# sandyresearch/chipmunk

Hardware: AMD Instinct MI355X
Metric: DiT denoise steps/sec at fixed sparsity (higher is better)
Workload: dtype bf16

## Files before the change

chipmunk_amd/csrc/attn96.hip:

```cpp
#include "common.h"
#include "attn64_regs.h"
#include "attn_params.h"
#include "attn64_util.h"
#include "attn96_sched.h"

namespace {

constexpr int KT = 32;
constexpr int TB = KT * 256;
constexpr int NSL = 4;
constexpr int VRING = NSL * TB;
constexpr int QLDS = 2 * NSL * TB;
constexpr int LDS_BYTES = QLDS + 2 * 8192;
constexpr float SCALE_LOG2E = 0.08838834764f * 1.44269504089f;
constexpr float MAX_LAG = 4.0f;
#ifndef A96_ABL
#define A96_ABL 0
#endif

template <int QB, int DB>
__device__ __forceinline__ void mfma_pv(const u32x4 &vf, const u32x4 &pf) {
    constexpr int oa = (QB * 4 + DB) * 16;
    asm volatile("s_nop 4\n\tv_mfma_f32_32x32x16_bf16 a[%c2:%c3], %0, %1, a[%c2:%c3]" ::"v"(vf), "v"(pf), "i"(oa), "i"(oa + 15));
}
template <int KS, int SLOT>
__device__ __forceinline__ void lds_k(uint32_t addr) {
    constexpr int ka = 192 + KS * 4;
    asm volatile("ds_read_b128 a[%c1:%c2], %0 offset:%c3" ::"v"(addr), "i"(ka), "i"(ka + 3), "i"(SLOT * TB) : "memory");
}

#ifdef ATTN96_PROF
__device__ unsigned long long g_a96_prof[2 * 8];
#define P96_DECL unsigned long long pt_ = 0, pacc_[7] = {0, 0, 0, 0, 0, 0, 0}; const bool prof_on_ = blockIdx.x == 700
#define P96_START() do { if (prof_on_) pt_ = __builtin_amdgcn_s_memtime(); } while (0)
#define P96_MARK(i) do { if (prof_on_) { const unsigned long long n_ = __builtin_amdgcn_s_memtime(); pacc_[i] += n_ - pt_; pt_ = n_; } } while (0)
#define P96_END(w, n) do { if (prof_on_ && lane == 0) { for (int i_ = 0; i_ < 7; ++i_) g_a96_prof[(w) * 8 + i_] = pacc_[i_]; g_a96_prof[(w) * 8 + 7] = (n); } } while (0)
#else
#define P96_DECL
#define P96_START()
#define P96_MARK(i)
#define P96_END(w, n)
#endif

template <bool INPLACE>
__global__ __launch_bounds__(128) __attribute__((amdgpu_waves_per_eu(1, 1))) void csp96_kernel(const AttnParams p) {
    extern __shared__ __attribute__((aligned(16))) unsigned char smem[];
    const int tid = threadIdx.x, lane = tid & 63;
    const int w = __builtin_amdgcn_readfirstlane(tid >> 6);
    const int l31 = lane & 31, hf = lane >> 5, l15 = lane & 15, lg = lane >> 4;
#ifdef ATTN96_PROF
    const unsigned long long t_entry_ = __builtin_amdgcn_s_memtime();
#endif
    int wid = blockIdx.x;
    const int wid0 = wid;
    wid = p.plan[2 * wid0];
    if (wid < 0) return;
    const int meta = p.plan[2 * wid0 + 1];
    const int sp = meta & 0xff, nsp = (meta >> 8) & 0xff;
    const int slot0 = meta >> 16, tix = meta >> 16;
    const int bh = wid / p.G, g = wid - bh * p.G;
    const int b = bh / p.H, h = bh - b * p.H;
    const int row0 = g * 192 + w * 96;
    const int count = p.counts[(int64_t)bh * p.G + g];
    const int valid = count < p.Nk ? count : p.Nk;
    const int ntiles_all = (valid + KT - 1) / KT;
    const int tbeg = (int)((int64_t)ntiles_all * sp / nsp), tend = (int)((int64_t)ntiles_all * (sp + 1) / nsp);
    const int ntiles = tend - tbeg;
    const int T4 = (ntiles + 3) & ~3;

    const uint16_t *kbase = p.k + b * p.ks[0] + h * p.ks[1];
    const uint16_t *vbase = p.v + b * p.vs[0] + h * p.vs[1];
    const __amdgpu_buffer_rsrc_t krsrc = make_rsrc(kbase), vrsrc = make_rsrc(vbase);
    const uint32_t kstride_b = (uint32_t)p.ks[2] * 2u, vstride_b = (uint32_t)p.vs[2] * 2u;
    const IndexRow irow = index_row(p, (int64_t)bh * p.G + g);
    const int32_t *idx = irow.ptr;

    const uint32_t lds0 = (uint32_t)(uintptr_t)(__attribute__((address_space(3))) unsigned char *)smem;
    uint32_t kad[8];
#pragma unroll
    for (int ks = 0; ks < 8; ++ks) kad[ks] = lds0 + l31 * 256 + (((2 * ks + hf) ^ l15) << 4);
    const uint32_t qad = lds0 + QLDS + w * 8192 + l31 * 256;
    uint32_t vad[4];
#pragma unroll
    for (int db = 0; db < 4; ++db)
        vad[db] = lds0 + VRING + (4 * hf + (l15 >> 2)) * 256 + (((db * 4 + 2 * (lg & 1) + ((l15 & 3) >> 1)) ^ ((l15 >> 2) << 2)) << 4) +
                  (l15 & 1) * 8;
    uint32_t kswz[4];
#pragma unroll
    for (int i = 0; i < 4; ++i) kswz[i] = (uint32_t)(l15 ^ (4 * i + lg)) << 4;
    const uint32_t vswz = (uint32_t)(l15 ^ (lg << 2)) << 4;
    const __amdgpu_buffer_rsrc_t irsrc = __builtin_amdgcn_make_buffer_rsrc((void *)idx, 0, irow.width * 4, 0x00020000);
    const int nk1 = p.Nk - 1;
    auto load_idx = [&](int T) {
        const int base = ((tbeg + T) * KT + w * 16 + lg * 4) * 4;
        u32x4 v4 = __builtin_amdgcn_raw_buffer_load_b128(irsrc, base, 0, 0);
        return v4;
    };
    auto clamp_idx = [&](u32x4 &v4) {
#pragma unroll
        for (int e = 0; e < 4; ++e)
            asm("v_med3_i32 %0, %1, 0, %2" : "=v"(v4[e]) : "v"(v4[e]), "v"(nk1));
    };
    auto issue_k1 = [&](const u32x4 &keys, int slot, int i) {
        blds16(krsrc, __umul24(keys[i], kstride_b) + kswz[i], 0, smem + slot * TB + (4 * w + i) * 1024);
    };
    auto issue_v1 = [&](const u32x4 &keys, int slot, int i) {
        blds16(vrsrc, __umul24(keys[i], vstride_b) + vswz, 0, smem + VRING + slot * TB + (4 * w + i) * 1024);
    };
    auto issue_k = [&](const u32x4 &keys, int slot) {
#pragma unroll
        for (int i = 0; i < 4; ++i) issue_k1(keys, slot, i);
    };
    auto issue_v = [&](const u32x4 &keys, int slot) {
#pragma unroll
        for (int i = 0; i < 4; ++i) issue_v1(keys, slot, i);
    };

    u32x4 ir[4];
    ir[0] = load_idx(0), ir[1] = load_idx(1), ir[2] = load_idx(2), ir[3] = load_idx(3);
    asm volatile(A96_ZERO_O ::: A64_CLOBBER_ALL);
    clamp_idx(ir[0]), clamp_idx(ir[1]), clamp_idx(ir[2]), clamp_idx(ir[3]);
    issue_k(ir[0], 0);
    issue_k(ir[1], 1), issue_v(ir[0], 3);
    issue_k(ir[2], 2), issue_v(ir[0], 0);
    issue_k(ir[3], 3), issue_v(ir[1], 1);
    ir[0] = load_idx(4);
    u32x4 qv[8];
    bool nomax = false;
    {
        const uint16_t *qp = p.q + b * p.qs[0] + h * p.qs[1];
        float qss[3] = {0.f, 0.f, 0.f};
        auto load_q = [&](auto foldc) {
            constexpr bool FOLD = decltype(foldc)::value != 0;
            static_for<0, 24>([&](auto f) {
                constexpr int F = decltype(f)::value, qb = F >> 3, ks = F & 7;
                const int qrow = row0 + qb * 32 + l31;
                u32x4 val = {0u, 0u, 0u, 0u};
                if (qrow < p.Nq) val = *(const u32x4 *)(qp + (int64_t)qrow * p.qs[2] + ks * 16 + hf * 8);
                if constexpr (FOLD) {
#pragma unroll
                    for (int e = 0; e < 4; ++e) {
                        const float lo = __uint_as_float(val[e] << 16), hi = __uint_as_float(val[e] & 0xffff0000u);
                        qss[qb] = __builtin_fmaf(lo, lo, qss[qb]);
                        qss[qb] = __builtin_fmaf(hi, hi, qss[qb]);
                        val[e] = pack_bf16x2(lo * SCALE_LOG2E, hi * SCALE_LOG2E);
                    }
                }
                if constexpr (qb == 0) qv[ks] = val;
                else if constexpr (qb == 2) acc_write4<224 + ks * 4>(val);
                else *(u32x4 *)(smem + QLDS + w * 8192 + l31 * 256 + (((2 * ks + hf) ^ l15) << 4)) = val;
            });
        };
        load_q(ic<1>{});
        if (p.kmax) {
            const float km = p.kmax[bh];
            bool ok = true;
#pragma unroll
            for (int qb = 0; qb < 3; ++qb) {
                float a = qss[qb], c2 = qss[qb];
                lane_swap32(a, c2);
                ok = ok && (__builtin_sqrtf(a + c2) * km * SCALE_LOG2E <= 55.0f);
            }
            nomax = __builtin_amdgcn_ballot_w64(!ok) == 0;
        }
        if (!nomax) load_q(ic<0>{});
    }

    asm volatile("s_waitcnt vmcnt(0)" ::: "memory");
    __syncthreads();
    static_for<0, 8>([&](auto i) { lds_k<decltype(i)::value, 0>(kad[decltype(i)::value]); });
    asm volatile("s_waitcnt lgkmcnt(0)" ::: "memory");

    f32x16 s[3];
#pragma unroll
    for (int q2 = 0; q2 < 3; ++q2)
#pragma unroll
        for (int r = 0; r < 16; ++r) s[q2][r] = -INFINITY;
#pragma unroll
    for (int r = 0; r < 7; ++r) s[1][r] = 0.f;
    u32x4 pw[3][2] = {};
    u32x4 pwo[2] = {};
    u32x2 vlo[4] = {}, vhi[4] = {};
    u32x4 q1w[4] = {};
    float m[3] = {-INFINITY, -INFINITY, -INFINITY}, nmsc[3] = {0.f, 0.f, 0.f}, mlag[3] = {-INFINITY, -INFINITY, -INFINITY};
    float lacc[3][2] = {{0.f, 0.f}, {0.f, 0.f}, {0.f, 0.f}};
    int vl_prev = KT;

    auto vhalf_read = [](uint32_t addr, auto offc, u32x2 &dst) __attribute__((always_inline)) {
        constexpr int OFF = decltype(offc)::value;
        asm volatile("ds_read_b64_tr_b16 %0, %1 offset:%c2" : "=v"(dst) : "v"(addr), "i"(OFF) : "memory");
    };
    auto q1_read = [&](auto ksc, u32x4 &dst) __attribute__((always_inline)) {
        constexpr int KS = decltype(ksc)::value;
        const uint32_t addr = qad + (kad[KS] - lds0 - l31 * 256);
        asm volatile("ds_read_b128 %0, %1" : "=v"(dst) : "v"(addr) : "memory");
    };
    auto mask_block = [&](f32x16 &sq, int vleft) __attribute__((always_inline)) {
        if (__builtin_expect(vleft < KT, 0)) {
            int thr = vleft - hf;
            asm volatile("" : "+v"(thr));
#pragma unroll
            for (int r = 0; r < 16; ++r)
                if ((r >> 3) * 16 + (r & 3) * 4 + 2 * ((r >> 2) & 1) >= thr) sq[r] = -INFINITY;
        }
    };
    auto max_step = [&](auto stepc, const f32x16 &sq, float &mx) __attribute__((always_inline)) {
        constexpr int K = decltype(stepc)::value, r0 = K * 4;
        if constexpr (K == 0)
            asm volatile("v_max_f32 %0, %1, %2\n\tv_max3_f32 %0, %0, %3, %4" : "=&v"(mx) : "v"(sq[0]), "v"(sq[1]), "v"(sq[2]), "v"(sq[3]));
        else
            asm volatile("v_max3_f32 %0, %0, %1, %2\n\tv_max3_f32 %0, %0, %3, %4" : "+v"(mx) : "v"(sq[r0]), "v"(sq[r0 + 1]), "v"(sq[r0 + 2]), "v"(sq[r0 + 3]));
    };
    auto max_halves = [&](float &mx) __attribute__((always_inline)) {
        float t0;
        asm volatile("v_mov_b32 %1, %0\n\ts_nop 1\n\tv_permlane32_swap_b32 %0, %1\n\ts_nop 0\n\tv_max_f32 %0, %0, %1" : "+v"(mx), "=&v"(t0));
    };
    auto update_block = [&](auto qq, float mx) __attribute__((always_inline)) {
        constexpr int QB = decltype(qq)::value;
        if (__builtin_expect(__builtin_amdgcn_ballot_w64(mx > mlag[QB]) != 0, 0)) {
            constexpr float LAG_RAW = MAX_LAG / SCALE_LOG2E;
            const float m_new = max2(m[QB], mx * SCALE_LOG2E);
            const float alpha = __builtin_amdgcn_exp2f(m[QB] - m_new);
            lacc[QB][0] *= alpha;
            lacc[QB][1] *= alpha;
            m[QB] = m_new;
            nmsc[QB] = -m_new;
            mlag[QB] = m_new * (1.0f / SCALE_LOG2E) + LAG_RAW;
            float tmp;
            if constexpr (QB == 0) asm volatile("s_nop 7\n\ts_nop 7\n\ts_nop 7\n\t" A96_SCALE_QB0 : "=&v"(tmp) : "v"(alpha));
            if constexpr (QB == 1) asm volatile("s_nop 7\n\ts_nop 7\n\ts_nop 7\n\t" A96_SCALE_QB1 : "=&v"(tmp) : "v"(alpha));
            if constexpr (QB == 2) asm volatile("s_nop 7\n\ts_nop 7\n\ts_nop 7\n\t" A96_SCALE_QB2 : "=&v"(tmp) : "v"(alpha));
        }
    };
    auto window = [&](auto qq, auto wc, auto nmc, auto parc) __attribute__((always_inline)) {
        constexpr int QB = decltype(qq)::value, W = decltype(wc)::value, PAR = decltype(parc)::value;
        constexpr bool NOMAX = decltype(nmc)::value != 0;
        if constexpr (W < 4 && !NOMAX) {
            static_for<4 * W, 4 * W + 4>([&](auto ee) {
                constexpr int E = decltype(ee)::value;
                float x = __builtin_fmaf(s[QB][E], SCALE_LOG2E, nmsc[QB]);
                pin(x);
                s[QB][E] = x;
            });
        }
        if constexpr (W >= 1 && W <= 16) {
#if A96_ABL & 16
            float e = s[QB][W - 1] * 0.5f;
#else
            float e = __builtin_amdgcn_exp2f(s[QB][W - 1]);
#endif
            pin(e);
            s[QB][W - 1] = e;
        }
        if constexpr (W >= 2 && W <= 17 && !(A96_ABL & 32)) {
            lacc[QB][W & 1] += s[QB][W - 2];
            pin(lacc[QB][W & 1]);
        }
        if constexpr (W >= 6 && W <= 20 && (W & 1) == 0) {
            constexpr int K = (W - 6) >> 1;
            uint32_t pk = pack_bf16x2(s[QB][2 * K], s[QB][2 * K + 1]);
            pin(pk);
            if constexpr (QB == 0 && PAR == 1) pwo[K >> 2][K & 3] = pk;
            else pw[QB][K >> 2][K & 3] = pk;
        }
    };

    P96_DECL;
    P96_START();
#ifdef ATTN96_PROF
    if (prof_on_) pacc_[2] = pt_ - t_entry_;
#endif
    auto tile = [&](auto slc, auto nmc, int t) __attribute__((always_inline)) {
        constexpr int SL = decltype(slc)::value;
        constexpr bool NOMAX = decltype(nmc)::value != 0;
        constexpr int VSL = (SL + 3) & 3;
        constexpr int KNSL = (SL + 1) & 3;
        if constexpr (!(A96_ABL & (4 | 128))) asm volatile("s_waitcnt vmcnt(18)" ::: "memory");
        if constexpr (!(A96_ABL & (4 | 64))) __builtin_amdgcn_s_barrier();
        P96_MARK(0);
        if constexpr (!(A96_ABL & 4)) ir[(SL + 1) & 3] = load_idx(t + 5);
        const int vl_cur = t < ntiles ? valid - (tbeg + t) * KT : 0;
        float mxa, mxb, mxc;
        __builtin_amdgcn_sched_barrier(0);
#ifdef A96_FORCE_MAJOR
        using S = a96s::Major;
#else
        using S = std::conditional_t<NOMAX, a96s::Pair, a96s::Major>;
#endif
        static_for<0, 48>([&](auto sg) {
            constexpr int SG = decltype(sg)::value;
#ifdef A96_TAILWAIT0
            if constexpr (SG == 1 || SG == 3 || SG == 5) asm volatile("s_waitcnt lgkmcnt(0)" ::: "memory");
            else
#endif
#ifdef A96_ALLWAIT0
            if constexpr ((SG & 1) == 1) asm volatile("s_waitcnt lgkmcnt(0)" ::: "memory");
            else
#endif
            if constexpr (S::WAIT[SG] >= 0 && !(A96_ABL & 2)) asm volatile("s_waitcnt lgkmcnt(%c0)" ::"i"(S::WAIT[SG]) : "memory");
            if constexpr ((SG & 1) == 0) {
                constexpr int qb = SG / 16, ks = (SG % 16) / 2, ka = 192 + ks * 4, qa = 224 + ks * 4;
                if constexpr (qb == 2) {
                    if constexpr (ks == 0) asm volatile("v_mfma_f32_32x32x16_bf16 %0, a[%c1:%c2], a[%c3:%c4], 0" : "=v"(s[2]) : "i"(ka), "i"(ka + 3), "i"(qa), "i"(qa + 3));
                    else asm volatile("v_mfma_f32_32x32x16_bf16 %0, a[%c1:%c2], a[%c3:%c4], %0" : "+v"(s[2]) : "i"(ka), "i"(ka + 3), "i"(qa), "i"(qa + 3));
                } else {
                    const u32x4 &qf = qb == 0 ? qv[ks] : q1w[ks & 3];
                    if constexpr (ks == 0) asm volatile("v_mfma_f32_32x32x16_bf16 %0, a[%c1:%c2], %3, 0" : "=v"(s[qb]) : "i"(ka), "i"(ka + 3), "v"(qf));
                    else asm volatile("v_mfma_f32_32x32x16_bf16 %0, a[%c1:%c2], %3, %0" : "+v"(s[qb]) : "i"(ka), "i"(ka + 3), "v"(qf));
                }
                if constexpr (SG % 4 == 2 && SG < 32 && !(A96_ABL & 4)) {
                    constexpr int PC = (SG - 2) / 4;
                    if constexpr (PC == 0) clamp_idx(ir[SL]);
                    if constexpr (PC < 4) issue_k1(ir[SL], SL, PC);
                    else issue_v1(ir[(SL + 2) & 3], (SL + 2) & 3, PC - 4);
                }
            } else {
                constexpr int I = (SG - 1) / 2, qbp = S::PV_QB[I], f = S::PV_F[I], e = S::PV_U[I], oa = (qbp * 4 + (f & 3)) * 16;
                const u32x4 vf = {vlo[e][0], vlo[e][1], vhi[e][0], vhi[e][1]};
                const u32x4 &pf = (qbp == 0 && ((SL + 1) & 1) == 1) ? pwo[f >> 2] : pw[qbp][f >> 2];
                asm volatile("v_mfma_f32_32x32x16_bf16 a[%c2:%c3], %0, %1, a[%c2:%c3]" ::"v"(vf), "v"(pf), "i"(oa), "i"(oa + 15));
            }
            static_for<0, 2>([&](auto jj) {
                constexpr int J = decltype(jj)::value;
                constexpr int kind = J == 0 ? S::RD_KIND0[SG] : S::RD_KIND1[SG], arg = J == 0 ? S::RD_ARG0[SG] : S::RD_ARG1[SG];
                if constexpr ((kind == 1 || kind == 2) && !(A96_ABL & 2)) {
                    constexpr int en = arg >> 3, fr = arg & 7, off = VSL * TB + (fr >> 2) * 4096 + (kind == 2 ? 2048 : 0);
                    vhalf_read(vad[fr & 3], ic<off>{}, kind == 1 ? vlo[en] : vhi[en]);
                }
                if constexpr (kind == 3 && !(A96_ABL & 8)) q1_read(ic<arg>{}, q1w[arg & 3]);
                if constexpr (kind == 4 && !(A96_ABL & 8)) lds_k<arg, KNSL>(kad[arg]);
            });
            if constexpr (!(A96_ABL & 1)) {
            if constexpr (SG == 0) mask_block(s[2], vl_prev);
            if constexpr (SG >= 1 && SG <= 4 && !NOMAX) max_step(ic<SG - 1>{}, s[2], mxc);
            if constexpr (SG == 5 && !NOMAX) max_halves(mxc);
            if constexpr (SG == 7 && !NOMAX) update_block(ic<2>{}, mxc);
            if constexpr (SG >= 8 && SG <= 31) window(ic<2>{}, ic<SG - 8>{}, nmc, ic<0>{});
            if constexpr (SG <= 15) window(ic<1>{}, ic<SG + 8>{}, nmc, ic<0>{});
            if constexpr (SG == 16) mask_block(s[0], vl_cur);
            if constexpr (SG >= 17 && SG <= 20 && !NOMAX) max_step(ic<SG - 17>{}, s[0], mxa);
            if constexpr (SG == 21 && !NOMAX) max_halves(mxa);
            if constexpr (SG == 23 && !NOMAX) update_block(ic<0>{}, mxa);
            if constexpr (SG >= 24) window(ic<0>{}, ic<SG - 24>{}, nmc, ic<(SL & 1)>{});
            if constexpr (SG == 32) mask_block(s[1], vl_cur);
            if constexpr (SG >= 33 && SG <= 36 && !NOMAX) max_step(ic<SG - 33>{}, s[1], mxb);
            if constexpr (SG == 37 && !NOMAX) max_halves(mxb);
            if constexpr (SG == 39 && !NOMAX) update_block(ic<1>{}, mxb);
            if constexpr (SG >= 40) window(ic<1>{}, ic<SG - 40>{}, nmc, ic<0>{});
            }
            __builtin_amdgcn_sched_barrier(0);
        });
        vl_prev = vl_cur;
        P96_MARK(1);
    };

    if (nomax) {
#pragma unroll
        for (int qb = 0; qb < 3; ++qb) m[qb] = 0.f, nmsc[qb] = 0.f, mlag[qb] = INFINITY;
    }
    if (nomax) {
        for (int tb = 0;; tb += 4) {
            tile(ic<0>{}, ic<1>{}, tb);
            if (tb >= T4) {
                asm volatile("s_waitcnt lgkmcnt(0)" ::: "memory");
                break;
            }
            tile(ic<1>{}, ic<1>{}, tb + 1);
            tile(ic<2>{}, ic<1>{}, tb + 2);
            tile(ic<3>{}, ic<1>{}, tb + 3);
        }
    } else {
        for (int tb = 0;; tb += 4) {
            tile(ic<0>{}, ic<0>{}, tb);
            if (tb >= T4) {
                asm volatile("s_waitcnt lgkmcnt(0)" ::: "memory");
                break;
            }
            tile(ic<1>{}, ic<0>{}, tb + 1);
            tile(ic<2>{}, ic<0>{}, tb + 2);
            tile(ic<3>{}, ic<0>{}, tb + 3);
        }
    }
    asm volatile("s_waitcnt lgkmcnt(0)" : "+v"(vlo[0]), "+v"(vhi[0]), "+v"(vlo[1]), "+v"(vhi[1]), "+v"(vlo[2]), "+v"(vhi[2]));
    mfma_pv<2, 1>((u32x4){vlo[0][0], vlo[0][1], vhi[0][0], vhi[0][1]}, pw[2][1]);
    mfma_pv<2, 2>((u32x4){vlo[1][0], vlo[1][1], vhi[1][0], vhi[1][1]}, pw[2][1]);
    mfma_pv<2, 3>((u32x4){vlo[2][0], vlo[2][1], vhi[2][0], vhi[2][1]}, pw[2][1]);
    asm volatile("s_waitcnt vmcnt(0)" ::: "memory");
#ifdef ATTN96_PROF
    const unsigned long long t_loop_end_ = __builtin_amdgcn_s_memtime();
#endif
    P96_END(w, T4 + 1);
    asm volatile("s_nop 7\n\ts_nop 7\n\ts_nop 7" ::: "memory");

    float lq[3];
#pragma unroll
    for (int qb = 0; qb < 3; ++qb) {
        float lp = lacc[qb][0] + lacc[qb][1], lo2 = lp;
        lane_swap32(lp, lo2);
        lq[qb] = lp + lo2;
    }
    auto read_o = [&](auto qq, float (&o)[64]) __attribute__((always_inline)) {
        constexpr int QB = decltype(qq)::value;
        static_for<0, 16>([&](auto ii) {
            constexpr int I = decltype(ii)::value;
            const f32x4 o4 = acc_read4<QB * 64 + I * 4>();
            o[I * 4 + 0] = o4[0], o[I * 4 + 1] = o4[1], o[I * 4 + 2] = o4[2], o[I * 4 + 3] = o4[3];
        });
    };
    auto load_base = [&](int qb, u32x2 (&old)[16]) __attribute__((always_inline)) {
        const int qrow = row0 + qb * 32 + l31;
        const int64_t ooff = b * p.os[0] + h * p.os[1] + (int64_t)qrow * p.os[2] + 4 * hf;
#pragma unroll
        for (int i = 0; i < 16; ++i) {
            const u32x2 z = {0u, 0u};
            old[i] = qrow < p.Nq ? *(const u32x2 *)(p.o_in + ooff + (i >> 2) * 32 + (i & 3) * 8) : z;
        }
    };
    auto store_o = [&](int qb, const float (&o)[64], float l, const u32x2 (&base)[16]) __attribute__((always_inline)) {
        const float inv = l > 0.f ? __builtin_amdgcn_rcpf(l) : 0.f;
        const int qrow = row0 + qb * 32 + l31;
        if (qrow >= p.Nq) return;
        const int64_t ooff = b * p.os[0] + h * p.os[1] + (int64_t)qrow * p.os[2] + 4 * hf;
#pragma unroll
        for (int i = 0; i < 16; ++i) {
            const int db = i >> 2, r4 = i & 3;
            const float *o4 = o + db * 16 + r4 * 4;
            const float x0 = o4[0] * inv, x1 = o4[1] * inv, x2 = o4[2] * inv, x3 = o4[3] * inv;
            u32x2 out;
            if constexpr (INPLACE) {
                const u32x2 old = base[i];
                const float a0 = round_bf16(x0 * p.o_scale), a1 = round_bf16(x1 * p.o_scale);
                const float a2 = round_bf16(x2 * p.o_scale), a3 = round_bf16(x3 * p.o_scale);
                out[0] = pack_bf16x2(__uint_as_float(old[0] << 16) + a0, __uint_as_float(old[0] & 0xffff0000u) + a1);
                out[1] = pack_bf16x2(__uint_as_float(old[1] << 16) + a2, __uint_as_float(old[1] & 0xffff0000u) + a3);
            } else {
                out[0] = pack_bf16x2(x0, x1);
                out[1] = pack_bf16x2(x2, x3);
            }
            *(u32x2 *)(p.o + ooff + db * 32 + r4 * 8) = out;
        }
    };

    if (nsp == 1) {
        constexpr int EP_I = 96 * 256 / 1024;
        const int er = lane >> 4, ech = lane & 15;
        const int64_t obase = b * p.os[0] + h * p.os[1];
        u32x4 base[EP_I] = {};
        if constexpr (INPLACE) {
#pragma unroll
            for (int j = 0; j < EP_I; ++j) {
                const int qrow = row0 + j * 4 + er;
                if (qrow < p.Nq) base[j] = *(const u32x4 *)(p.o_in + obase + (int64_t)qrow * p.os[2] + ech * 8);
            }
        }
        __syncthreads();
        unsigned char *stage = smem + w * (96 * 256);
        static_for<0, 3>([&](auto qq) {
            constexpr int QB = decltype(qq)::value;
            float o[64];
            read_o(qq, o);
            const float l = lq[QB];
            const float inv = (l > 0.f ? __builtin_amdgcn_rcpf(l) : 0.f) * (INPLACE ? p.o_scale : 1.f);
            const int r = QB * 32 + l31;
#pragma unroll
            for (int i = 0; i < 16; ++i) {
                const u32x2 out = {pack_bf16x2(o[i * 4 + 0] * inv, o[i * 4 + 1] * inv), pack_bf16x2(o[i * 4 + 2] * inv, o[i * 4 + 3] * inv)};
                *(u32x2 *)(stage + r * 256 + ((i ^ (r & 15)) << 4) + hf * 8) = out;
            }
        });
#pragma unroll
        for (int j = 0; j < EP_I; ++j) {
            const int r = j * 4 + er, qrow = row0 + r;
            if (qrow >= p.Nq) continue;
            u32x4 v = *(const u32x4 *)(stage + r * 256 + ((ech ^ (r & 15)) << 4));
            if constexpr (INPLACE) {
#pragma unroll
                for (int e = 0; e < 4; ++e)
                    v[e] = pack_bf16x2(__uint_as_float(base[j][e] << 16) + __uint_as_float(v[e] << 16),
                                       __uint_as_float(base[j][e] & 0xffff0000u) + __uint_as_float(v[e] & 0xffff0000u));
            }
            *(u32x4 *)(p.o + obase + (int64_t)qrow * p.os[2] + ech * 8) = v;
        }
#ifdef ATTN96_PROF
        asm volatile("s_waitcnt vmcnt(0)" ::: "memory");
        if (prof_on_ && lane == 0) g_a96_prof[w * 8 + 3] = __builtin_amdgcn_s_memtime() - t_loop_end_;
#endif
        return;
    }
    constexpr int SLICE_FLOATS = 26 * 256 * 4;
    int *ticket_s = (int *)smem;
    float *mine = p.ws + (int64_t)(slot0 + sp) * SLICE_FLOATS + tid;
    static_for<0, 3>([&](auto qq) {
        constexpr int QB = decltype(qq)::value;
        float o[64];
        read_o(qq, o);
#pragma unroll
        for (int i = 0; i < 64; ++i) mine[(QB * 64 + i) * 128] = o[i];
        mine[(192 + QB) * 128] = m[QB];
        mine[(195 + QB) * 128] = lq[QB];
    });
    __syncthreads();
    if (tid == 0) {
        __builtin_amdgcn_fence(__ATOMIC_RELEASE, "agent");
        asm volatile("s_waitcnt vmcnt(0)" ::: "memory");
        *ticket_s = __hip_atomic_fetch_add(p.tickets + tix, 1, __ATOMIC_RELAXED, __HIP_MEMORY_SCOPE_AGENT);
    }
    __syncthreads();
    if (*ticket_s != nsp - 1) return;
    if (tid == 0) {
        __hip_atomic_store(p.tickets + tix, 0, __ATOMIC_RELAXED, __HIP_MEMORY_SCOPE_AGENT);
        __builtin_amdgcn_fence(__ATOMIC_ACQUIRE, "agent");
    }
    __syncthreads();
#pragma unroll 1
    for (int qb = 0; qb < 3; ++qb) {
        float o[64];
#pragma unroll
        for (int i = 0; i < 64; ++i) o[i] = 0.f;
        float mm = -INFINITY, ll = 0.f;
        for (int s2 = 0; s2 < nsp; ++s2) {
            const float *oth = p.ws + (int64_t)(slot0 + s2) * SLICE_FLOATS + tid;
            const float ms = oth[(192 + qb) * 128], ls = oth[(195 + qb) * 128];
            const float m_new = fmaxf(mm, ms);
            if (m_new == -INFINITY) continue;
            const float a = __builtin_amdgcn_exp2f(mm - m_new);
            const float c = __builtin_amdgcn_exp2f(ms - m_new);
            mm = m_new;
            ll = ll * a + ls * c;
#pragma unroll
            for (int i = 0; i < 64; ++i) o[i] = o[i] * a + oth[(qb * 64 + i) * 128] * c;
        }
        u32x2 base[16] = {};
        if constexpr (INPLACE) load_base(qb, base);
        store_o(qb, o, ll, base);
    }
}

template <bool INPLACE>
int launch96(const AttnParams &p, int grid, hipStream_t stream) {
    auto kern = csp96_kernel<INPLACE>;
    static uint64_t lds_set = 0;
    ensure_dynamic_lds((const void *)kern, LDS_BYTES, lds_set);
    hipLaunchKernelGGL(kern, dim3((unsigned)grid), dim3(128), LDS_BYTES, stream, p);
    CM_LAUNCH_CHECK();
    return CHIPMUNK_OK;
}

}

#ifdef ATTN96_PROF
extern "C" int chipmunk_attn96_prof_read(unsigned long long *out) {
    return hipMemcpyFromSymbol(out, HIP_SYMBOL(g_a96_prof), sizeof(g_a96_prof)) == hipSuccess ? 0 : 2;
}
#endif

int chipmunk_csp96_launch(const AttnParams &p, int inplace, int grid, hipStream_t stream) {
    CM_CHECK(p.plan && p.tickets && p.ws, "csp96: work plan missing");
    AttnParams pp = p;
    pp.kmax = chipmunk_knorm_max(p.k, p.ks, p.B, p.H, p.Nk, stream);
    return inplace ? launch96<true>(pp, grid, stream) : launch96<false>(pp, grid, stream);
}
```

chipmunk_amd/csrc/attn96_sched.h:

```cpp
#pragma once
namespace a96s {
struct Pair {
    static constexpr int PV_QB[24] = {2, 2, 2, 0, 1, 0, 1, 0, 1, 0, 1, 0, 1, 0, 1, 0, 1, 0, 1, 2, 2, 2, 2, 2};
    static constexpr int PV_F[24] = {5, 6, 7, 0, 0, 1, 1, 2, 2, 3, 3, 4, 4, 5, 5, 6, 6, 7, 7, 0, 1, 2, 3, 4};
    static constexpr int PV_U[24] = {0, 1, 2, 3, 3, 0, 0, 1, 1, 2, 2, 3, 3, 0, 0, 1, 1, 2, 2, 3, 0, 1, 2, 3};
    static constexpr int RD_KIND0[48] = {1, 2, 3, 0, 1, 2, 3, 0, 1, 2, 3, 0, 1, 2, 3, 0, 1, 2, 3, 3, 1, 2, 3, 3, 1, 2, 1, 2, 1, 2, 1, 2, 0, 4, 1, 2, 0, 4, 1, 2, 1, 2, 1, 2, 1, 2, 1, 2};
    static constexpr int RD_ARG0[48] = {24, 24, 0, 0, 1, 1, 1, 0, 10, 10, 2, 0, 19, 19, 3, 0, 28, 28, 4, 5, 5, 5, 6, 7, 14, 14, 24, 24, 23, 23, 1, 1, 0, 0, 10, 10, 0, 2, 19, 19, 28, 28, 5, 5, 14, 14, 23, 23};
    static constexpr int RD_KIND1[48] = {0, 0, 0, 0, 0, 0, 0, 0, 0, 0, 0, 0, 0, 0, 0, 0, 0, 0, 0, 0, 0, 0, 0, 0, 0, 0, 0, 0, 0, 0, 0, 0, 0, 0, 0, 4, 0, 0, 0, 4, 0, 4, 0, 4, 0, 4, 0, 4};
    static constexpr int RD_ARG1[48] = {0, 0, 0, 0, 0, 0, 0, 0, 0, 0, 0, 0, 0, 0, 0, 0, 0, 0, 0, 0, 0, 0, 0, 0, 0, 0, 0, 0, 0, 0, 0, 0, 0, 0, 0, 1, 0, 0, 0, 3, 0, 4, 0, 5, 0, 6, 0, 7};
    static constexpr int WAIT[48] = {-1, 8, -1, 7, -1, 5, -1, 4, -1, -1, -1, 4, -1, -1, -1, 4, -1, -1, -1, 4, -1, -1, 6, 5, 5, -1, 6, 5, 5, -1, 6, 5, -1, -1, -1, 4, -1, -1, -1, -1, -1, 9, -1, 9, -1, 8, -1, 8};
};
struct Major {
    static constexpr int PV_QB[24] = {2, 2, 2, 0, 0, 0, 0, 0, 0, 0, 0, 1, 1, 1, 1, 1, 1, 1, 1, 2, 2, 2, 2, 2};
    static constexpr int PV_F[24] = {5, 6, 7, 0, 1, 2, 3, 4, 5, 6, 7, 0, 1, 2, 3, 4, 5, 6, 7, 0, 1, 2, 3, 4};
    static constexpr int PV_U[24] = {0, 1, 2, 3, 0, 1, 2, 3, 0, 1, 2, 3, 0, 1, 2, 3, 0, 1, 2, 3, 0, 1, 2, 3};
    static constexpr int RD_KIND0[48] = {1, 2, 1, 2, 1, 2, 1, 2, 1, 2, 1, 2, 1, 2, 1, 2, 1, 2, 1, 2, 1, 2, 1, 2, 1, 2, 1, 2, 1, 2, 1, 2, 1, 2, 1, 2, 1, 2, 1, 2, 1, 2, 1, 2, 1, 2, 1, 2};
    static constexpr int RD_ARG0[48] = {24, 24, 1, 1, 10, 10, 19, 19, 28, 28, 5, 5, 14, 14, 23, 23, 24, 24, 1, 1, 10, 10, 19, 19, 28, 28, 5, 5, 14, 14, 23, 23, 24, 24, 1, 1, 10, 10, 19, 19, 28, 28, 5, 5, 14, 14, 23, 23};
    static constexpr int RD_KIND1[48] = {0, 0, 3, 0, 0, 0, 3, 0, 0, 0, 3, 0, 0, 0, 3, 0, 0, 0, 3, 3, 0, 0, 3, 3, 0, 0, 0, 0, 0, 0, 0, 0, 0, 4, 0, 4, 0, 4, 0, 4, 0, 4, 0, 4, 0, 4, 0, 4};
    static constexpr int RD_ARG1[48] = {0, 0, 0, 0, 0, 0, 1, 0, 0, 0, 2, 0, 0, 0, 3, 0, 0, 0, 4, 5, 0, 0, 6, 7, 0, 0, 0, 0, 0, 0, 0, 0, 0, 0, 0, 1, 0, 2, 0, 3, 0, 4, 0, 5, 0, 6, 0, 7};
    static constexpr int WAIT[48] = {-1, 8, -1, 8, -1, 7, -1, 7, -1, 6, -1, 7, -1, 6, -1, 7, -1, 6, -1, 7, -1, 7, -1, 8, 8, 8, 8, 7, 6, 6, 6, 5, -1, 5, -1, 6, -1, 7, -1, 8, -1, 8, -1, 8, -1, 8, -1, 8};
};
}
```

Baseline: 0.5902.

## Keep second Q block in VGPRs instead of re-reading from LDS each tile

The second 32-row Q block is now held in eight VGPR vectors for the whole kernel, so the per-tile ds_read_b128 of Q from LDS is gone. That frees the Q region of LDS and shrinks the LDS footprint. K-fragment LDS addresses are now built on the fly with an XOR from a single base, with a few precomputed in the no-max path, instead of being kept as eight registers. The read schedules and lgkm wait counts are retuned to match the fewer LDS reads. The cost is higher VGPR pressure, which could cause spills or worse scheduling, and the new wait counts must stay correct.

```diff
diff --git a/chipmunk_amd/csrc/attn96.hip b/chipmunk_amd/csrc/attn96.hip
--- a/chipmunk_amd/csrc/attn96.hip
+++ b/chipmunk_amd/csrc/attn96.hip
@@ -10,10 +10,10 @@
 constexpr int TB = KT * 256;
 constexpr int NSL = 4;
 constexpr int VRING = NSL * TB;
-constexpr int QLDS = 2 * NSL * TB;
-constexpr int LDS_BYTES = QLDS + 2 * 8192;
+constexpr int LDS_BYTES = 2 * NSL * TB;
 constexpr float SCALE_LOG2E = 0.08838834764f * 1.44269504089f;
 constexpr float MAX_LAG = 4.0f;
+constexpr int NKR = 4;
 #ifndef A96_ABL
 #define A96_ABL 0
 #endif
@@ -44,7 +44,7 @@
 
 template <bool INPLACE>
 __global__ __launch_bounds__(128) __attribute__((amdgpu_waves_per_eu(1, 1))) void csp96_kernel(const AttnParams p) {
-    extern __shared__ __attribute__((aligned(16))) unsigned char smem[];
+    extern __shared__ __attribute__((aligned(256))) unsigned char smem[];
     const int tid = threadIdx.x, lane = tid & 63;
     const int w = __builtin_amdgcn_readfirstlane(tid >> 6);
     const int l31 = lane & 31, hf = lane >> 5, l15 = lane & 15, lg = lane >> 4;
@@ -76,10 +76,7 @@
     const int32_t *idx = irow.ptr;
 
     const uint32_t lds0 = (uint32_t)(uintptr_t)(__attribute__((address_space(3))) unsigned char *)smem;
-    uint32_t kad[8];
-#pragma unroll
-    for (int ks = 0; ks < 8; ++ks) kad[ks] = lds0 + l31 * 256 + (((2 * ks + hf) ^ l15) << 4);
-    const uint32_t qad = lds0 + QLDS + w * 8192 + l31 * 256;
+    const uint32_t kad0 = lds0 + l31 * 256 + ((hf ^ l15) << 4);
     uint32_t vad[4];
 #pragma unroll
     for (int db = 0; db < 4; ++db)
@@ -99,7 +96,7 @@
     auto clamp_idx = [&](u32x4 &v4) {
 #pragma unroll
         for (int e = 0; e < 4; ++e)
-            asm("v_med3_i32 %0, %1, 0, %2" : "=v"(v4[e]) : "v"(v4[e]), "v"(nk1));
+            asm("v_med3_i32 %0, %1, 0, %2" : "=v"(v4[e]) : "v"(v4[e]), "s"(nk1));
     };
     auto issue_k1 = [&](const u32x4 &keys, int slot, int i) {
         blds16(krsrc, __umul24(keys[i], kstride_b) + kswz[i], 0, smem + slot * TB + (4 * w + i) * 1024);
@@ -125,7 +122,7 @@
     issue_k(ir[2], 2), issue_v(ir[0], 0);
     issue_k(ir[3], 3), issue_v(ir[1], 1);
     ir[0] = load_idx(4);
-    u32x4 qv[8];
+    u32x4 qv[8], q1v[8];
     bool nomax = false;
     {
         const uint16_t *qp = p.q + b * p.qs[0] + h * p.qs[1];
@@ -148,7 +145,7 @@
                 }
                 if constexpr (qb == 0) qv[ks] = val;
                 else if constexpr (qb == 2) acc_write4<224 + ks * 4>(val);
-                else *(u32x4 *)(smem + QLDS + w * 8192 + l31 * 256 + (((2 * ks + hf) ^ l15) << 4)) = val;
+                else q1v[ks] = val;
             });
         };
         load_q(ic<1>{});
@@ -168,7 +165,7 @@
 
     asm volatile("s_waitcnt vmcnt(0)" ::: "memory");
     __syncthreads();
-    static_for<0, 8>([&](auto i) { lds_k<decltype(i)::value, 0>(kad[decltype(i)::value]); });
+    static_for<0, 8>([&](auto i) { lds_k<decltype(i)::value, 0>(kad0 ^ (decltype(i)::value << 5)); });
     asm volatile("s_waitcnt lgkmcnt(0)" ::: "memory");
 
     f32x16 s[3];
@@ -181,7 +178,6 @@
     u32x4 pw[3][2] = {};
     u32x4 pwo[2] = {};
     u32x2 vlo[4] = {}, vhi[4] = {};
-    u32x4 q1w[4] = {};
     float m[3] = {-INFINITY, -INFINITY, -INFINITY}, nmsc[3] = {0.f, 0.f, 0.f}, mlag[3] = {-INFINITY, -INFINITY, -INFINITY};
     float lacc[3][2] = {{0.f, 0.f}, {0.f, 0.f}, {0.f, 0.f}};
     int vl_prev = KT;
@@ -189,11 +185,6 @@
     auto vhalf_read = [](uint32_t addr, auto offc, u32x2 &dst) __attribute__((always_inline)) {
         constexpr int OFF = decltype(offc)::value;
         asm volatile("ds_read_b64_tr_b16 %0, %1 offset:%c2" : "=v"(dst) : "v"(addr), "i"(OFF) : "memory");
-    };
-    auto q1_read = [&](auto ksc, u32x4 &dst) __attribute__((always_inline)) {
-        constexpr int KS = decltype(ksc)::value;
-        const uint32_t addr = qad + (kad[KS] - lds0 - l31 * 256);
-        asm volatile("ds_read_b128 %0, %1" : "=v"(dst) : "v"(addr) : "memory");
     };
     auto mask_block = [&](f32x16 &sq, int vleft) __attribute__((always_inline)) {
         if (__builtin_expect(vleft < KT, 0)) {
@@ -265,6 +256,8 @@
         }
     };
 
+    uint32_t kadn[NKR];
+    kadn[0] = kad0;
     P96_DECL;
     P96_START();
 #ifdef ATTN96_PROF
@@ -280,6 +273,7 @@
         P96_MARK(0);
         if constexpr (!(A96_ABL & 4)) ir[(SL + 1) & 3] = load_idx(t + 5);
         const int vl_cur = t < ntiles ? valid - (tbeg + t) * KT : 0;
+        uint32_t kt = kad0;
         float mxa, mxb, mxc;
         __builtin_amdgcn_sched_barrier(0);
 #ifdef A96_FORCE_MAJOR
@@ -304,7 +298,7 @@
                     if constexpr (ks == 0) asm volatile("v_mfma_f32_32x32x16_bf16 %0, a[%c1:%c2], a[%c3:%c4], 0" : "=v"(s[2]) : "i"(ka), "i"(ka + 3), "i"(qa), "i"(qa + 3));
                     else asm volatile("v_mfma_f32_32x32x16_bf16 %0, a[%c1:%c2], a[%c3:%c4], %0" : "+v"(s[2]) : "i"(ka), "i"(ka + 3), "i"(qa), "i"(qa + 3));
                 } else {
-                    const u32x4 &qf = qb == 0 ? qv[ks] : q1w[ks & 3];
+                    const u32x4 &qf = qb == 0 ? qv[ks] : q1v[ks];
                     if constexpr (ks == 0) asm volatile("v_mfma_f32_32x32x16_bf16 %0, a[%c1:%c2], %3, 0" : "=v"(s[qb]) : "i"(ka), "i"(ka + 3), "v"(qf));
                     else asm volatile("v_mfma_f32_32x32x16_bf16 %0, a[%c1:%c2], %3, %0" : "+v"(s[qb]) : "i"(ka), "i"(ka + 3), "v"(qf));
                 }
@@ -320,6 +314,10 @@
                 const u32x4 &pf = (qbp == 0 && ((SL + 1) & 1) == 1) ? pwo[f >> 2] : pw[qbp][f >> 2];
                 asm volatile("v_mfma_f32_32x32x16_bf16 a[%c2:%c3], %0, %1, a[%c2:%c3]" ::"v"(vf), "v"(pf), "i"(oa), "i"(oa + 15));
             }
+            if constexpr (SG + 1 < 48) {
+                constexpr int karg = S::RD_KIND0[SG + 1] == 4 ? S::RD_ARG0[SG + 1] : S::RD_KIND1[SG + 1] == 4 ? S::RD_ARG1[SG + 1] : 0;
+                if constexpr (karg >= (NOMAX ? NKR : 1)) asm volatile("v_xor_b32 %0, %c2, %1" : "=v"(kt) : "v"(kad0), "i"(karg << 5));
+            }
             static_for<0, 2>([&](auto jj) {
                 constexpr int J = decltype(jj)::value;
                 constexpr int kind = J == 0 ? S::RD_KIND0[SG] : S::RD_KIND1[SG], arg = J == 0 ? S::RD_ARG0[SG] : S::RD_ARG1[SG];
@@ -327,8 +325,10 @@
                     constexpr int en = arg >> 3, fr = arg & 7, off = VSL * TB + (fr >> 2) * 4096 + (kind == 2 ? 2048 : 0);
                     vhalf_read(vad[fr & 3], ic<off>{}, kind == 1 ? vlo[en] : vhi[en]);
                 }
-                if constexpr (kind == 3 && !(A96_ABL & 8)) q1_read(ic<arg>{}, q1w[arg & 3]);
-                if constexpr (kind == 4 && !(A96_ABL & 8)) lds_k<arg, KNSL>(kad[arg]);
+                if constexpr (kind == 4 && !(A96_ABL & 8)) {
+                    if constexpr (arg < (NOMAX ? NKR : 1)) lds_k<arg, KNSL>(kadn[arg]);
+                    else lds_k<arg, KNSL>(kt);
+                }
             });
             if constexpr (!(A96_ABL & 1)) {
             if constexpr (SG == 0) mask_block(s[2], vl_prev);
@@ -359,6 +359,8 @@
         for (int qb = 0; qb < 3; ++qb) m[qb] = 0.f, nmsc[qb] = 0.f, mlag[qb] = INFINITY;
     }
     if (nomax) {
+#pragma unroll
+        for (int ks = 1; ks < NKR; ++ks) kadn[ks] = kad0 ^ (ks << 5);
         for (int tb = 0;; tb += 4) {
             tile(ic<0>{}, ic<1>{}, tb);
             if (tb >= T4) {
diff --git a/chipmunk_amd/csrc/attn96_sched.h b/chipmunk_amd/csrc/attn96_sched.h
--- a/chipmunk_amd/csrc/attn96_sched.h
+++ b/chipmunk_amd/csrc/attn96_sched.h
@@ -4,11 +4,11 @@
     static constexpr int PV_QB[24] = {2, 2, 2, 0, 1, 0, 1, 0, 1, 0, 1, 0, 1, 0, 1, 0, 1, 0, 1, 2, 2, 2, 2, 2};
     static constexpr int PV_F[24] = {5, 6, 7, 0, 0, 1, 1, 2, 2, 3, 3, 4, 4, 5, 5, 6, 6, 7, 7, 0, 1, 2, 3, 4};
     static constexpr int PV_U[24] = {0, 1, 2, 3, 3, 0, 0, 1, 1, 2, 2, 3, 3, 0, 0, 1, 1, 2, 2, 3, 0, 1, 2, 3};
-    static constexpr int RD_KIND0[48] = {1, 2, 3, 0, 1, 2, 3, 0, 1, 2, 3, 0, 1, 2, 3, 0, 1, 2, 3, 3, 1, 2, 3, 3, 1, 2, 1, 2, 1, 2, 1, 2, 0, 4, 1, 2, 0, 4, 1, 2, 1, 2, 1, 2, 1, 2, 1, 2};
-    static constexpr int RD_ARG0[48] = {24, 24, 0, 0, 1, 1, 1, 0, 10, 10, 2, 0, 19, 19, 3, 0, 28, 28, 4, 5, 5, 5, 6, 7, 14, 14, 24, 24, 23, 23, 1, 1, 0, 0, 10, 10, 0, 2, 19, 19, 28, 28, 5, 5, 14, 14, 23, 23};
+    static constexpr int RD_KIND0[48] = {1, 2, 0, 0, 1, 2, 0, 0, 1, 2, 0, 0, 1, 2, 0, 0, 1, 2, 0, 0, 1, 2, 0, 0, 1, 2, 1, 2, 1, 2, 1, 2, 0, 4, 1, 2, 0, 4, 1, 2, 1, 2, 1, 2, 1, 2, 1, 2};
+    static constexpr int RD_ARG0[48] = {24, 24, 0, 0, 1, 1, 0, 0, 10, 10, 0, 0, 19, 19, 0, 0, 28, 28, 0, 0, 5, 5, 0, 0, 14, 14, 24, 24, 23, 23, 1, 1, 0, 0, 10, 10, 0, 2, 19, 19, 28, 28, 5, 5, 14, 14, 23, 23};
     static constexpr int RD_KIND1[48] = {0, 0, 0, 0, 0, 0, 0, 0, 0, 0, 0, 0, 0, 0, 0, 0, 0, 0, 0, 0, 0, 0, 0, 0, 0, 0, 0, 0, 0, 0, 0, 0, 0, 0, 0, 4, 0, 0, 0, 4, 0, 4, 0, 4, 0, 4, 0, 4};
     static constexpr int RD_ARG1[48] = {0, 0, 0, 0, 0, 0, 0, 0, 0, 0, 0, 0, 0, 0, 0, 0, 0, 0, 0, 0, 0, 0, 0, 0, 0, 0, 0, 0, 0, 0, 0, 0, 0, 0, 0, 1, 0, 0, 0, 3, 0, 4, 0, 5, 0, 6, 0, 7};
-    static constexpr int WAIT[48] = {-1, 8, -1, 7, -1, 5, -1, 4, -1, -1, -1, 4, -1, -1, -1, 4, -1, -1, -1, 4, -1, -1, 6, 5, 5, -1, 6, 5, 5, -1, 6, 5, -1, -1, -1, 4, -1, -1, -1, -1, -1, 9, -1, 9, -1, 8, -1, 8};
+    static constexpr int WAIT[48] = {-1, 8, -1, 6, -1, 4, -1, 2, -1, -1, -1, 2, -1, -1, -1, 2, -1, -1, -1, 2, -1, -1, -1, 2, -1, -1, -1, 3, -1, -1, -1, 5, -1, -1, -1, 4, -1, -1, -1, -1, -1, 9, -1, 9, -1, 8, -1, 8};
 };
 struct Major {
     static constexpr int PV_QB[24] = {2, 2, 2, 0, 0, 0, 0, 0, 0, 0, 0, 1, 1, 1, 1, 1, 1, 1, 1, 2, 2, 2, 2, 2};
@@ -16,8 +16,8 @@
     static constexpr int PV_U[24] = {0, 1, 2, 3, 0, 1, 2, 3, 0, 1, 2, 3, 0, 1, 2, 3, 0, 1, 2, 3, 0, 1, 2, 3};
     static constexpr int RD_KIND0[48] = {1, 2, 1, 2, 1, 2, 1, 2, 1, 2, 1, 2, 1, 2, 1, 2, 1, 2, 1, 2, 1, 2, 1, 2, 1, 2, 1, 2, 1, 2, 1, 2, 1, 2, 1, 2, 1, 2, 1, 2, 1, 2, 1, 2, 1, 2, 1, 2};
     static constexpr int RD_ARG0[48] = {24, 24, 1, 1, 10, 10, 19, 19, 28, 28, 5, 5, 14, 14, 23, 23, 24, 24, 1, 1, 10, 10, 19, 19, 28, 28, 5, 5, 14, 14, 23, 23, 24, 24, 1, 1, 10, 10, 19, 19, 28, 28, 5, 5, 14, 14, 23, 23};
-    static constexpr int RD_KIND1[48] = {0, 0, 3, 0, 0, 0, 3, 0, 0, 0, 3, 0, 0, 0, 3, 0, 0, 0, 3, 3, 0, 0, 3, 3, 0, 0, 0, 0, 0, 0, 0, 0, 0, 4, 0, 4, 0, 4, 0, 4, 0, 4, 0, 4, 0, 4, 0, 4};
-    static constexpr int RD_ARG1[48] = {0, 0, 0, 0, 0, 0, 1, 0, 0, 0, 2, 0, 0, 0, 3, 0, 0, 0, 4, 5, 0, 0, 6, 7, 0, 0, 0, 0, 0, 0, 0, 0, 0, 0, 0, 1, 0, 2, 0, 3, 0, 4, 0, 5, 0, 6, 0, 7};
-    static constexpr int WAIT[48] = {-1, 8, -1, 8, -1, 7, -1, 7, -1, 6, -1, 7, -1, 6, -1, 7, -1, 6, -1, 7, -1, 7, -1, 8, 8, 8, 8, 7, 6, 6, 6, 5, -1, 5, -1, 6, -1, 7, -1, 8, -1, 8, -1, 8, -1, 8, -1, 8};
+    static constexpr int RD_KIND1[48] = {0, 0, 0, 0, 0, 0, 0, 0, 0, 0, 0, 0, 0, 0, 0, 0, 0, 0, 0, 0, 0, 0, 0, 0, 0, 0, 0, 0, 0, 0, 0, 0, 0, 4, 0, 4, 0, 4, 0, 4, 0, 4, 0, 4, 0, 4, 0, 4};
+    static constexpr int RD_ARG1[48] = {0, 0, 0, 0, 0, 0, 0, 0, 0, 0, 0, 0, 0, 0, 0, 0, 0, 0, 0, 0, 0, 0, 0, 0, 0, 0, 0, 0, 0, 0, 0, 0, 0, 0, 0, 1, 0, 2, 0, 3, 0, 4, 0, 5, 0, 6, 0, 7};
+    static constexpr int WAIT[48] = {-1, 8, -1, 7, -1, 6, -1, 5, -1, 5, -1, 5, -1, 5, -1, 5, -1, 5, -1, 5, -1, 5, -1, 5, -1, 5, -1, 5, -1, 5, -1, 5, -1, 5, -1, 6, -1, 7, -1, 8, -1, 8, -1, 8, -1, 8, -1, 8};
 };
 }
```

Result: no change. 0.5934, median of 6 (+0.6%).
